# TorbenHellriegel/Speaker-Recognition-x-vectors

Hardware: AMD Instinct MI355X
Metric: x-vector embeddings/sec (300-frame utt) (higher is better)
Workload: dtype f32; 1 GPU; configs[1]: 1xMI355X batch=256 fixed 300-frame x 24-MFCC utterances, fp32 frame-level stack, extract_x_vec layer 6, random-init weights seed 42; build=xvec_hip gfx950 build a1dbbf885613, batch_per_gpu=256, frames=300

## Files before the change

### speaker-recognition-x-vectors_amd/csrc/tdnn_layer_impl.h

```cpp
#pragma once
#include <cstdlib>

#include "tdnn_common.h"

namespace xvec {

constexpr int kBM = 128, kBN = 128;
constexpr int kStageFloats = (kBM + kBN) * kBK;
constexpr int kConstFloats = 3 * kBN;
constexpr int kLdsBytes = (2 * kStageFloats + kConstFloats) * 4;

#ifdef XVEC_DIAG
static __device__ unsigned long long g_diag[8 * 8192];
#endif

struct Ctx {
    __amdgpu_buffer_rsrc_t xrsrc;
    __amdgpu_buffer_rsrc_t wrsrc;
    int x_base;
    int ur0, ur1, ur2, ur3;
    int xo0, xo1, xo2, xo3;
    int w_toff;
    __amdgpu_buffer_rsrc_t wfrsrc;
    int wf_voff;
// ... 218 lines not shown
    }

#define XV_CHUNK3(P_, N_, IT_)                                                                            \
    {                                                                                                     \
        const float* S = smem + P_ * kStageFloats;                                                        \
        const float* Sn = smem + N_ * kStageFloats;                                                       \
        XV_G3(0, gb0_0, XV_FRG_L(0, 0, S), XV_FRG_L(1, 0, S), XV_FRG_L(2, 0, S), XV_FRG_L(3, 0, S))       \
        XV_G3(0, gb0_1, XV_LST3(0, N_), XV_LST3(1, N_), XV_LST3(2, N_), XV_LST3(3, N_))                   \
        XV_G3(1, gb0_0, XV_FRG_A(0, 1, 0, S), XV_FRG_A(1, 1, 0, S), XV_FRG_A(2, 1, 0, S),                 \
              XV_FRG_A(3, 1, 0, S))                                                                       \
        XV_ADVANCE                                                                                        \
        XV_G3(0, gb1_0, XV_FRG_L(0, 1, S), XV_FRG_L(1, 1, S), XV_FRG_L(2, 1, S), XV_FRG_L(3, 1, S))       \
        XV_G3(0, gb1_1, XV_GLB3(0, (IT_) + 1), XV_GLD_A(0, 0) XV_GLD_A(1, 0),                             \
              XV_GLD_A(2, 0) XV_GLD_A(3, 0), XV_GLD_B(0, 0) XV_GLD_B(1, 0))                               \
        XV_G3(1, gb1_0, XV_FRG_A(0, 2, 0, S), XV_FRG_A(1, 2, 0, S), XV_FRG_A(2, 2, 0, S),                 \
              XV_FRG_A(3, 2, 0, S))                                                                       \
        XV_G3(0, gb2_0, XV_FRG_L(0, 2, S), XV_FRG_L(1, 2, S), XV_FRG_L(2, 2, S), XV_FRG_L(3, 2, S))       \
        XV_G3(0, gb2_1, XV_GLB3(1, (IT_) + 1), XV_GLD_B(2, 0) XV_GLD_B(3, 0), XV_NOP, XV_NOP)             \
        XV_G3(1, gb2_0, XV_FRG_A(0, 3, 0, S), XV_FRG_A(1, 3, 0, S), XV_FRG_A(2, 3, 0, S),                 \
              XV_FRG_A(3, 3, 0, S))                                                                       \
        XV_G3(0, gb3_0, XV_FRG_L(0, 3, S), XV_FRG_L(1, 3, S), XV_FRG_L(2, 3, S), XV_FRG_L(3, 3, S))       \
        XV_G3(0, gb3_1, XV_GLB3(2, (IT_) + 1), XV_NOP, XV_NOP, XV_NOP)                                    \
        __syncthreads();                      \
        XV_G3(1, gb3_0, XV_FRG_A(0, 0, 0, Sn), XV_FRG_A(1, 0, 0, Sn), XV_FRG_A(2, 0, 0, Sn),              \
              XV_FRG_A(3, 0, 0, Sn))                                                                      \
        XV_GLB3(3, (IT_) + 1)                                                                             \
    }

struct Regs {
    float4 sA0_0, sA1_0, sA2_0, sA3_0, sB0_0, sB1_0, sB2_0, sB3_0;
    float4 sA0_1, sA1_1, sA2_1, sA3_1, sB0_1, sB1_1, sB2_1, sB3_1;
    float4 fa0_0, fa1_0, fa2_0, fa3_0, fb_0, fa0_1, fa1_1, fa2_1, fa3_1, fb_1;
    float4 gb0_0, gb1_0, gb2_0, gb3_0, gb0_1, gb1_1, gb2_1, gb3_1;
    float4 w3[2][6];
};

struct Lane {
    int h, sw, a_rd, b_rd, st_off, r0, c, col;
    int st3, rd3;
};

constexpr int kPlaneBytes = kBM * kBK * 2;

__device__ __forceinline__ void s3_store(char* B, int st3, int i, const float4& v) {
    u32x2 hi, mid, lo;
    split3(v, hi, mid, lo);
    *reinterpret_cast<u32x2*>(B + st3 + i * 32 * 64) = hi;
    *reinterpret_cast<u32x2*>(B + kPlaneBytes + st3 + i * 32 * 64) = mid;
    *reinterpret_cast<u32x2*>(B + 2 * kPlaneBytes + st3 + i * 32 * 64) = lo;
}

template <int NG>
__device__ __forceinline__ void s3_gld(const TdnnArgs& a, const Ctx& cx, float4& d0, float4& d1, float4& d2, float4& d3) {
    const int soff = ((cx.tap * a.tap_rows) * a.ldx + cx.kc * kBK) * 4;
    const int rs = 32 * a.ldx * 4;
    if constexpr (NG > 0) d0 = buf_load16(cx.xrsrc, cx.xo0, soff);
    if constexpr (NG > 1) d1 = buf_load16(cx.xrsrc, cx.xo1, soff + rs);
    if constexpr (NG > 2) d2 = buf_load16(cx.xrsrc, cx.xo2, soff + 2 * rs);
    if constexpr (NG > 3) d3 = buf_load16(cx.xrsrc, cx.xo3, soff + 3 * rs);
}

__device__ __forceinline__ void s3_wld(const Ctx& cx, float4* w, int c, int n_chunks) {
    if (c >= n_chunks) c -= n_chunks;
#pragma unroll
    for (int j = 0; j < 6; ++j) w[j] = buf_load16(cx.wfrsrc, cx.wf_voff, (6 * c + j) * 1024);
}

#define XV_S3_CHUNK(P_, N_, IT_)                                                                          \
    {                                                                                                     \
        const char* S = reinterpret_cast<const char*>(smem) + P_ * kStageFloats * 4;                      \
        char* Sn = reinterpret_cast<char*>(smem) + N_ * kStageFloats * 4;                                 \
        if constexpr (G > 0) s3_store(Sn, ln.st3, 0, rg.sA0_##N_);                                         \
        if constexpr (G > 1) s3_store(Sn, ln.st3, 1, rg.sA1_##N_);                                         \
        if constexpr (G > 2) s3_store(Sn, ln.st3, 2, rg.sA2_##N_);                                         \
        if constexpr (G > 3) s3_store(Sn, ln.st3, 3, rg.sA3_##N_);                                         \
        advance<GUARD, false>(a, cx, n_chunks);                                                           \
        s3_gld<G>(a, cx, rg.sA0_##N_, rg.sA1_##N_, rg.sA2_##N_, rg.sA3_##N_);                              \
        s3_wld(cx, rg.w3[N_], (IT_) + 1, n_chunks);                                                       \
        _Pragma("unroll") for (int s3 = 0; s3 < 2; ++s3) {                                                \
            const int rd = ln.rd3 ^ (32 * s3);                                                            \
            float4 xf[4][3];                                                                              \
            _Pragma("unroll") for (int i = 0; i < G; ++i)                                                 \
                _Pragma("unroll") for (int pl = 0; pl < 3; ++pl)                                          \
                    xf[i][pl] = *reinterpret_cast<const float4*>(S + pl * kPlaneBytes + i * 32 * 64 + rd); \
            if constexpr (G > 0) s3_mfma6(acc0, xf[0], rg.w3[P_] + 3 * s3);                                \
            if constexpr (G > 1) s3_mfma6(acc1, xf[1], rg.w3[P_] + 3 * s3);                                \
            if constexpr (G > 2) s3_mfma6(acc2, xf[2], rg.w3[P_] + 3 * s3);                                \
            if constexpr (G > 3) s3_mfma6(acc3, xf[3], rg.w3[P_] + 3 * s3);                                \
        }                                                                                                 \
        __syncthreads();                      \
    }

template <int GUARD, bool INBF, bool X3, bool S3>
__device__ __forceinline__ void block_prologue(const TdnnArgs& a, float* smem, Ctx& cx, Regs& rg, const Lane& ln,
                                               int n_chunks) {
    constexpr int G = 4;
    constexpr int ES = INBF ? 2 : 4, BKE = 128 / ES;
    const int h = ln.h, sw = ln.sw, a_rd = ln.a_rd, b_rd = ln.b_rd, st_off = ln.st_off, c = ln.c;
    if constexpr (S3) {
        char* B0 = reinterpret_cast<char*>(smem);
        s3_gld<4>(a, cx, rg.sA0_0, rg.sA1_0, rg.sA2_0, rg.sA3_0);
        advance<GUARD, false>(a, cx, n_chunks);
        s3_gld<4>(a, cx, rg.sA0_1, rg.sA1_1, rg.sA2_1, rg.sA3_1);
        s3_wld(cx, rg.w3[0], 0, n_chunks);
        s3_store(B0, ln.st3, 0, rg.sA0_0);
        s3_store(B0, ln.st3, 1, rg.sA1_0);
        s3_store(B0, ln.st3, 2, rg.sA2_0);
        s3_store(B0, ln.st3, 3, rg.sA3_0);
        advance<GUARD, false>(a, cx, n_chunks);
        s3_gld<4>(a, cx, rg.sA0_0, rg.sA1_0, rg.sA2_0, rg.sA3_0);
        __syncthreads();
        return;
    }
    if constexpr (X3) {
        XV_GLD_ALL(0)
        SB();
        XV_LST3(0, 0) XV_LST3(1, 0) XV_LST3(2, 0) XV_LST3(3, 0)
        SB();
        advance<GUARD, X3>(a, cx, n_chunks);
        XV_GLD_ALL(0)
    } else {
        XV_GLD_ALL(0)
        advance<GUARD, X3>(a, cx, n_chunks);
        XV_GLD_ALL(1)
        SB();
        XV_LST_ALL(0)
        SB();
        advance<GUARD, X3>(a, cx, n_chunks);
        XV_GLD_ALL(0)
    }
    __syncthreads();
    XV_FRG_A(0, 0, 0, smem) XV_FRG_A(1, 0, 0, smem) XV_FRG_A(2, 0, 0, smem) XV_FRG_A(3, 0, 0, smem)
    XV_FRG_B(0, 0, smem)
    XV_GLB(0, 0, 0) XV_GLB(1, 0, 0) XV_GLB(2, 0, 0) XV_GLB(3, 0, 0)
    XV_GLB(0, 1, 1) XV_GLB(1, 1, 1) XV_GLB(2, 1, 1) XV_GLB(3, 1, 1)
    XV_GLB3(0, 0) XV_GLB3(1, 0) XV_GLB3(2, 0) XV_GLB3(3, 0)
    SB();
}

template <int G, int GUARD, bool POOL, bool STORE, bool INBF, bool OUTBF, bool X3, bool S3>
__device__ __forceinline__ void process_tile(const TdnnArgs& a, float* smem, Ctx& cx, Regs& rg, const Lane& ln,
                                             int64_t g0, int n0, int n_chunks) {
    constexpr int ES = INBF ? 2 : 4, BKE = 128 / ES;
    const int h = ln.h, sw = ln.sw, a_rd = ln.a_rd, b_rd = ln.b_rd, st_off = ln.st_off, c = ln.c;
    constexpr bool SWAP = INBF && OUTBF && !X3 && STORE && !POOL;
    f32x16 acc0, acc1, acc2, acc3;
    const float* cstw = smem + 2 * kStageFloats + (ln.col - n0 - (int)(threadIdx.x & 31)) + 4 * ln.h;
    if constexpr (SWAP) {
#pragma unroll
        for (int gq = 0; gq < 4; ++gq) {
            const float4 b4 = *reinterpret_cast<const float4*>(cstw + 8 * gq);
            acc0[4 * gq] = b4.x; acc0[4 * gq + 1] = b4.y; acc0[4 * gq + 2] = b4.z; acc0[4 * gq + 3] = b4.w;
        }
        acc1 = acc0; acc2 = acc0; acc3 = acc0;
    } else if constexpr (POOL) {
        const float b0 = smem[2 * kStageFloats + kBN + (ln.col - n0)];
#pragma unroll
        for (int e = 0; e < 16; ++e) acc0[e] = b0;
        acc1 = acc0; acc2 = acc0; acc3 = acc0;
    } else {
#pragma unroll
        for (int e = 0; e < 16; ++e) { acc0[e] = 0.f; acc1[e] = 0.f; acc2[e] = 0.f; acc3[e] = 0.f; }
    }

#ifdef XVEC_DIAG
    SB();
    const unsigned long long dt0 = __builtin_amdgcn_s_memtime();
    SB();
#endif
    for (int it = 0; it < n_chunks; it += 2) {
        if constexpr (S3) {
            XV_S3_CHUNK(0, 1, it)
            XV_S3_CHUNK(1, 0, it + 1)
        } else if constexpr (X3) {
            XV_CHUNK3(0, 1, it)
            XV_CHUNK3(1, 0, it + 1)
        } else {
            XV_CHUNK(0, 1, it)
            XV_CHUNK(1, 0, it + 1)
        }
    }
#ifdef XVEC_DIAG
    SB();
    const unsigned long long dt1 = __builtin_amdgcn_s_memtime();
    SB();
#endif

    const int64_t m0 = g0 * 32;
    const int col = ln.col;
    float* cst = smem + 2 * kStageFloats + (col - n0);
    const float bi = cst[0], sc = cst[kBN], sh = cst[2 * kBN];
    float negk = sh;
    if constexpr (POOL) {
        if (!cx.pivot_set) {
            const float piv = lower_half(fmaxf(acc0[0] + bi, 0.f));
            const float bmk = bi - piv;
            negk = bmk - bi;
#pragma unroll
            for (int e = 0; e < 16; ++e) {
                acc0[e] += bmk;
                if constexpr (G > 1) acc1[e] += bmk;
                if constexpr (G > 2) acc2[e] += bmk;
                if constexpr (G > 3) acc3[e] += bmk;
            }
            cst[kBN] = bmk;
            cst[2 * kBN] = negk;
            cx.pivot_set = true;
        }
    }
    const int esz = OUTBF ? 2 : 4;
    __amdgpu_buffer_rsrc_t yrsrc;
    int y_voff = 0;
    __amdgpu_buffer_rsrc_t yrsrc_lo;
    if (STORE) {
        yrsrc = make_rsrc(static_cast<char*>(a.Y) + (m0 * (int64_t)a.ldy + n0) * esz);
        if constexpr (X3 && OUTBF)
            yrsrc_lo = make_rsrc(static_cast<char*>(a.Y) + a.y_plane_bytes + (m0 * (int64_t)a.ldy + n0) * esz);
        y_voff = (4 * h * a.ldy + (col - n0)) * esz;
    }
#define XV_EPI(i_)                                                                                        \
    if constexpr (G > i_) {                                                                               \
                                                                                       \
        if constexpr (!POOL) {                                                                            \
            _Pragma("unroll") for (int e = 0; e < 16; ++e)                                                \
                acc##i_[e] = fmaf(fmaxf(acc##i_[e] + bi, 0.f), sc, sh);                                   \
            asm volatile("" : "+v"(acc##i_));                                                             \
        }                                                                                                 \
        if (STORE) {                                                                                      \
            _Pragma("unroll") for (int e = 0; e < 16; ++e) {                                              \
                const int soff = (i_ * 32 + (e & 3) + 8 * (e >> 2)) * a.ldy * esz;                        \
// ... 43 lines not shown
    }
#endif
}

template <int GUARD, bool POOL, bool STORE, bool INBF, bool OUTBF, bool X3, bool S3>
__device__ __forceinline__ void tdnn_body(const TdnnArgs& a, float* smem) {
#ifdef XVEC_DIAG
    const unsigned long long t_entry = __builtin_amdgcn_s_memtime(), r_entry = __builtin_amdgcn_s_memrealtime();
    if (threadIdx.x == 0 && blockIdx.x < 8192) { g_diag[blockIdx.x * 8 + 3] = 0; g_diag[blockIdx.x * 8 + 4] = 0; g_diag[blockIdx.x * 8 + 5] = 0; }
#endif
    const int lid = xcd_remap(blockIdx.x, gridDim.x);
    const int j = lid % a.n_tiles;
    const int p = lid / a.n_tiles;
    int64_t g_begin, g_end;
    group_range(a, p, g_begin, g_end);
    const int n0 = j * kBN;
    const int n_chunks = a.n_taps * a.cpt;

    const int tid = threadIdx.x;
    const int lane = tid & 63, wave = tid >> 6;
    Lane ln;
    ln.h = lane >> 5;
    const int r = lane & 31;
    ln.c = tid & 7;
    ln.r0 = tid >> 3;
    ln.st_off = ln.r0 * kBK + ((ln.c ^ ((ln.r0 >> 1) & 7)) << 2);
    ln.sw = (r >> 1) & 7;
    ln.a_rd = r * kBK;
    ln.b_rd = kBM * kBK + (wave * 32 + r) * kBK;
    ln.col = n0 + wave * 32 + r;
    ln.st3 = ln.r0 * 64 + ((((ln.c >> 1) ^ ((ln.r0 >> 2) & 3)) * 16) | ((ln.c & 1) * 8));
    ln.rd3 = r * 64 + ((ln.h ^ ((r >> 2) & 3)) * 16);
    if (tid < kBN) {
        smem[2 * kStageFloats + tid] = a.bias[n0 + tid];
        smem[2 * kStageFloats + kBN + tid] = POOL ? 0.f : a.scale[n0 + tid];
        smem[2 * kStageFloats + 2 * kBN + tid] = POOL ? 0.f : a.shift[n0 + tid];
    }

    Ctx cx;
    cx.g_s = g_begin;
    cx.g_end = g_end;
    cx.m0 = g_begin * 32;
    constexpr int ES = INBF ? 2 : 4;
    cx.es = ES;
    cx.xrsrc = x_rsrc<GUARD>(a, cx);
    cx.wrsrc = make_rsrc(static_cast<const char*>(a.W) + (int64_t)n0 * a.k_pad * ES);
    cx.x_base = ln.r0 * a.ldx * ES + ln.c * 16;
    cx.w_toff = ln.r0 * a.k_pad * ES + ln.c * 16;
    cx.r0 = ln.r0;
    if (INBF) {
        const int64_t ct = n0 / 32 + wave;
        cx.wfrsrc = make_rsrc(static_cast<const char*>(a.Wf) + ct * (int64_t)(a.k_pad / 16) * 1024);
        cx.wf_voff = lane * 16;
    }
    if (S3) {
        const int64_t ct = n0 / 32 + wave;
        cx.wfrsrc = make_rsrc(static_cast<const char*>(a.Wf) + ct * (int64_t)(a.k_pad / 16) * 3072);
        cx.wf_voff = lane * 16;
    }
    cx.u_tile = __builtin_amdgcn_readfirstlane(utt_of_row(a.out_map, cx.m0));
    cx.off_next = row_off(a.out_map, cx.u_tile + 1);
    if (POOL) {
        cx.pool.u = cx.u_tile;
        cx.pool.end = cx.off_next;
    }
    cx.pivot_set = false;
    set_tile_rows(a, cx);
    cx.tap = 0;
    cx.kc = 0;
    cx.itl = 0;

    Regs rg;
    block_prologue<GUARD, INBF, X3, S3>(a, smem, cx, rg, ln, n_chunks);
    int64_t g = g_begin;
    for (; g + 4 <= g_end; g += 4) process_tile<4, GUARD, POOL, STORE, INBF, OUTBF, X3, S3>(a, smem, cx, rg, ln, g, n0, n_chunks);
    const int rem = (int)(g_end - g);
    if (rem == 3) process_tile<3, GUARD, POOL, STORE, INBF, OUTBF, X3, S3>(a, smem, cx, rg, ln, g, n0, n_chunks);
    else if (rem == 2) process_tile<2, GUARD, POOL, STORE, INBF, OUTBF, X3, S3>(a, smem, cx, rg, ln, g, n0, n_chunks);
    else if (rem == 1) process_tile<1, GUARD, POOL, STORE, INBF, OUTBF, X3, S3>(a, smem, cx, rg, ln, g, n0, n_chunks);
#ifdef XVEC_DIAG
    if (threadIdx.x == 0 && blockIdx.x < 8192) {
        __builtin_amdgcn_s_waitcnt(0);
        unsigned long long* d = g_diag + blockIdx.x * 8;
        d[0] = t_entry;
        d[1] = __builtin_amdgcn_s_memtime();
        d[2] = (unsigned long long)(g_end - g_begin);
        d[6] = r_entry;
        d[7] = __builtin_amdgcn_s_memrealtime();
    }
#endif
}

template <typename K>
static hipError_t launch_kernel(K kern, const TdnnArgs& a, hipStream_t s, LdsOptIn& opt) {
    if (a.groups_total <= 0 || a.blocks_per_col <= 0 || a.blocks_per_col > a.groups_total || (a.cpt & 1))
        return hipErrorInvalidValue;
    if (hipError_t e = opt.ensure(reinterpret_cast<const void*>(kern), kLdsBytes); e != hipSuccess) return e;
    const int grid = a.blocks_per_col * a.n_tiles;
    kern<<<dim3(grid), dim3(256), kLdsBytes, s>>>(a);
    return hipGetLastError();
}

}
```

### speaker-recognition-x-vectors_amd/csrc/tdnn_split3.hip

```cpp
#include "tdnn_layer_impl.h"

namespace xvec {

template <bool POOL, bool STORE>
__global__ __launch_bounds__(256, 2) void tdnn_split3_kernel(const TdnnArgs a) {
    extern __shared__ __attribute__((aligned(16))) float smem[];
    tdnn_body<false, POOL, STORE, false, false, false, true>(a, smem);
}

hipError_t launch_tdnn_split3(const TdnnArgs& a, bool pool, hipStream_t s) {
    static LdsOptIn opt_store, opt_pool;
    if (a.n_taps != 1) return hipErrorInvalidValue;
    return pool ? launch_kernel(tdnn_split3_kernel<true, false>, a, s, opt_pool)
                : launch_kernel(tdnn_split3_kernel<false, true>, a, s, opt_store);
}

}
```

### speaker-recognition-x-vectors_amd/csrc/xvec_api.hip

```cpp
#include <hip/hip_runtime.h>

#include <algorithm>
#include <cstdio>
#include <cstdlib>
#include <cstring>
#include <new>

#include "../../include/xvec_hip.h"
#include "host_support.h"
#include "pool_segments.h"
#include "tdnn_common.h"
#include "xvec_internal.h"

using namespace xvec;

namespace {

thread_local ErrorChannel g_err;

#define HIP_TRY(expr)                                                                         \
    do {                                                                                      \
        hipError_t e_ = (expr);                                                               \
        if (e_ != hipSuccess)                                                                 \
            return g_err.fail(XVEC_ERR_HIP, "%s failed: %s (%s:%d)", #expr,                   \
                              hipGetErrorString(e_), __FILE__, __LINE__);                     \
    } while (0)

const int kCtxLen[XVEC_NUM_TDNN] = {5, 3, 3, 1, 1};
const int kCtxDil[XVEC_NUM_TDNN] = {1, 2, 3, 0, 0};

enum { T_L1 = 0, T_POOL = 5, T_SEG6 = 6, T_SEG7 = 7, T_OUT = 8, T_PACK = 9, T_COUNT = 10 };
constexpr int kMaxUtts = 65535;
constexpr int kSplit3MinRowsPerCu = 64;
constexpr int kWinoS3MinRowsPerCu = 64;

struct Policy {
    int blocks_per_cu;
    bool pp;
    int pp_min_tenths;
    int pp_cu_pct;
    bool wino;
    bool split3;
    int split3_min_rows;
    bool wino_split3;
    int wino_s3_min_rows;
};

int env_int(const char* name, int unset) {
    const char* e = getenv(name);
    return e ? atoi(e) : unset;
}

Policy read_policy() {
    const int tenths = env_int("XVEC_PP_MIN_TENTHS", 18), s3_rows = env_int("XVEC_SPLIT3_MIN_ROWS", kSplit3MinRowsPerCu);
    const int ws3_rows = env_int("XVEC_WINO_SPLIT3_MIN_ROWS", kWinoS3MinRowsPerCu);
    return {std::max(1, env_int("XVEC_BLOCKS_PER_CU", 2)), env_int("XVEC_PP", 1) != 0, tenths > 0 ? tenths : 18,
            env_int("XVEC_PP_CU_PCT", 0), env_int("XVEC_WINOGRAD", 1) != 0, env_int("XVEC_SPLIT3", 1) != 0,
            s3_rows >= 0 ? s3_rows : kSplit3MinRowsPerCu, env_int("XVEC_WINO_SPLIT3", 1) != 0,
            ws3_rows >= 0 ? ws3_rows : kWinoS3MinRowsPerCu};
}

struct DeviceGuard {
    int prev = -1;
    bool changed = false;
    hipError_t enter(int dev) {
        hipError_t e = hipGetDevice(&prev);
        if (e != hipSuccess) return e;
        if (prev != dev) {
            e = hipSetDevice(dev);
            changed = e == hipSuccess;
        }
        return e;
    }
    ~DeviceGuard() {
        if (changed) (void)hipSetDevice(prev);
    }
};

}

struct xvec_handle {
    xvec_cfg cfg;
    int cin_pad;
    TdnnGeom geo[XVEC_NUM_TDNN];
    TdnnGeom geo16[XVEC_NUM_TDNN];
    void* Wp16[XVEC_NUM_TDNN];
    void* Wp16b;
    void* Wr16[XVEC_NUM_TDNN];
    void* Wp48[XVEC_NUM_TDNN];
    void* Wr48[XVEC_NUM_TDNN];
    float* Wp[XVEC_NUM_TDNN];
    float* Wu[XVEC_NUM_TDNN];
    void* Wu3[XVEC_NUM_TDNN];
    void* Wp3[XVEC_NUM_TDNN];
    float* vec[XVEC_NUM_TDNN];
    float* Wraw[XVEC_NUM_TDNN];
    float* braw[XVEC_NUM_TDNN];
    float* vec16[XVEC_NUM_TDNN];
    bool folded[XVEC_NUM_TDNN];
    hipEvent_t load_evt[XVEC_NUM_TDNN];
    bool tdnn_loaded[XVEC_NUM_TDNN];
    float* affW[3];
    float* affB[3];
    void* affW3[3];
    int affN[3], affK[3];
    bool aff_loaded[3];
    int64_t* offs_pinned[2];
    hipEvent_t offs_evt[2];
    bool offs_pending[2];
    int offs_next;
    int num_cu;
    Policy pol;
    int last_kernel[XVEC_NUM_TDNN];
    int last_form[XVEC_NUM_TDNN];
    int last_operands[XVEC_NUM_TDNN];
    int last_aff_form[3];
    int last_aff_ranges[3];
    bool profiling;
    hipEvent_t ev0[T_COUNT], ev1[T_COUNT];
    bool ev_used[T_COUNT];
};

namespace {

struct Plan {
    int64_t total, m_pad, rows_alloc;
    size_t xpad, x16, actA, actB, act5, part, part_cnt, pooled, seg6, seg7, offs, bytes;
    int64_t part_slots;
};


Plan make_plan(const xvec_handle* h, int64_t total, int B) {
    Plan p;
    p.total = total;
    p.m_pad = round_up64(total > 0 ? total : 1, 128);
    p.rows_alloc = p.m_pad + kRowPadTail;
    const int nh = h->geo[0].n_pad, n5 = h->geo[4].n_pad;
    size_t o = 0;
    p.xpad = o;   o += align256((size_t)p.rows_alloc * h->cin_pad * 4);
    p.x16 = o;    o += align256((size_t)p.rows_alloc * h->cin_pad * 2 * 2);
    p.actA = o;   o += align256((size_t)p.rows_alloc * nh * 4);
    p.actB = o;   o += align256((size_t)p.rows_alloc * nh * 4);
    p.act5 = o;   o += align256((size_t)p.rows_alloc * (n5 > nh ? n5 : nh) * 4);
    p.part_slots = std::max<int64_t>(p.m_pad / 32 + B + 1, 2 * ((int64_t)h->num_cu + B) + 2);
// ... 57 lines not shown
    for (int i = 0; i < 3; ++i) {
        f(&h->affW[i], (size_t)h->affN[i] * h->affK[i] * 4);
        f(&h->affB[i], (size_t)h->affN[i] * 4);
        f(&h->affW3[i], h->affK[i] % 4 == 0 ? (size_t)h->affN[i] * h->affK[i] * 4 : 0);
    }
}

int aff_index(int which) { return which == XVEC_SEG6 ? 0 : which == XVEC_SEG7 ? 1 : which == XVEC_OUTPUT ? 2 : -1; }

struct StageTimer {
    xvec_handle* h;
    int idx;
    hipStream_t s;
    StageTimer(xvec_handle* h_, int idx_, hipStream_t s_) : h(h_), idx(idx_), s(s_) {
        if (h->profiling) (void)hipEventRecord(h->ev0[idx], s);
    }
    ~StageTimer() {
        if (h->profiling) {
            (void)hipEventRecord(h->ev1[idx], s);
            h->ev_used[idx] = true;
        }
    }
};

int pp_blocks_per_col(const xvec_handle* h, int n_pad, int64_t rows_out) {
    const Policy& pol = h->pol;
    if (!pol.pp || n_pad % 256 != 0) return 0;
    int bpc = h->num_cu / (n_pad / 256);
    if (pol.pp_cu_pct > 0 && pol.pp_cu_pct < 100) bpc = (bpc * pol.pp_cu_pct + 50) / 100;
    const int64_t units = (rows_out + 63) / 64;
    return (bpc >= 1 && units >= bpc && 10 * units >= pol.pp_min_tenths * (int64_t)bpc) ? bpc : 0;
}

void persistent_grid(const xvec_handle* h, int n_tiles, int64_t groups_total, int* blocks_per_col, int* pair_period) {
    const int per_col = (int)std::max<int64_t>(1, std::min<int64_t>((int64_t)h->num_cu * h->pol.blocks_per_cu / n_tiles, groups_total));
    const int nwg = per_col * n_tiles;
    const bool ok = h->pol.blocks_per_cu == 2 && nwg == 2 * h->num_cu && nwg % 16 == 0 && (nwg / 8) % (2 * n_tiles) == 0;
    *blocks_per_col = per_col;
    *pair_period = ok ? (nwg / 8) / n_tiles : 0;
}

struct LayerCall {
    int layer;
    TdnnMode mode;
    const void* X;
    int ldx;
    int64_t x_rows;
    void* X16;
    int64_t x_plane, y_plane;
    void* Y;
    float* part;
    int* part_cnt;
    RowMap map;
    int64_t rows_out;
};

enum class Launch { kDirect, kPp16, kFirst, kFirst3, kSplit3, kWino, kWinoS3 };

struct LayerPlan {
    int layer;
    Launch launch;
    int kernel, form;
    int operands;
    TdnnMode mode;
    TdnnArgs a;
    int64_t pool_units;
    int pool_bpc;
};

int plan_layer(const xvec_handle* h, const LayerCall& c, LayerPlan& lp) {
    const int l = c.layer;
    const bool bf = c.mode.prec != Prec::kF32, x3 = c.mode.prec == Prec::kBf16x3, pool = c.mode.dst == Dst::kPool;
    const bool from_act = c.mode.src == Src::kAct;
    const TdnnGeom& g = bf ? h->geo16[l] : h->geo[l];
    memset(&lp, 0, sizeof(lp));
    lp.layer = l;
    lp.mode = c.mode;
    lp.kernel = XVEC_KERNEL_TILE128;
    lp.form = XVEC_FORM_DIRECT;
    lp.operands = !bf ? XVEC_OPERANDS_FP32 : x3 ? XVEC_OPERANDS_BF16X3 : XVEC_OPERANDS_BF16;
    TdnnArgs& a = lp.a;
    a.X = c.X;
    a.W = h->Wp[l];
    a.Wf = x3 ? h->Wp48[l] : h->Wp16[l];
    const float* vecs = (bf && !x3) ? h->vec16[l] : h->vec[l];
    a.bias = vecs;
    a.scale = vecs + g.n_pad;
    a.shift = vecs + 2 * g.n_pad;
    a.Y = c.Y;
    a.x_rows = c.x_rows;
    a.ldx = c.ldx;
    a.ldy = g.n_pad;
    a.n_taps = g.n_taps;
    a.tap_rows = g.tap_rows;
    a.kpt = g.kpt;
    a.cpt = g.kpt_pad / (bf ? 2 * kBK : kBK);
    a.k_pad = x3 ? 2 * g.k_pad : g.k_pad;
    a.n_tiles = g.n_pad / 128;
    a.groups_total = (c.rows_out + 31) / 32;
    persistent_grid(h, a.n_tiles, a.groups_total, &a.blocks_per_col, &a.pair_period);
    a.pool_part = c.part;
    a.pool_cnt = c.part_cnt;
    a.out_map = c.map;
    a.span = h->geo[l].ctx_span;
    a.terms = x3 ? 2 : 1;
    a.y_plane_bytes = x3 ? (int)c.y_plane : 0;
    int bpc = 0;
    if (bf && l > 0 && from_act && c.mode.dst != Dst::kF32 && (bpc = pp_blocks_per_col(h, g.n_pad, c.rows_out))) {
        lp.launch = Launch::kPp16;
        lp.kernel = XVEC_KERNEL_PP;
        a.W = x3 ? h->Wr48[l] : h->Wr16[l];
        a.n_tiles = g.n_pad / 256;
        a.blocks_per_col = lp.pool_bpc = bpc;
        a.groups_total = lp.pool_units = (c.rows_out + 63) / 64;
        a.pair_period = 0;
    } else if (bf && l == 0 && !from_act && c.mode.dst == Dst::kAct && h->pol.pp &&
               (x3 ? tdnn_first3_applicable(a) : tdnn_first_applicable(a))) {
        lp.launch = x3 ? Launch::kFirst3 : Launch::kFirst;
        lp.kernel = XVEC_KERNEL_FIRST;
        if (!x3) a.Wf = h->Wp16b;
    } else if (x3 && c.mode.src == Src::kRows32) {
        if (!c.X16) return g_err.fail(XVEC_ERR_STATE, "internal: bf16x3 layer 1 from fp32 rows needs the streaming kernel's shapes");
        lp.mode.src = Src::kRows16;
        a.X = c.X16;
    } else if (!bf && from_act && h->pol.split3 && h->Wp3[l] && c.rows_out >= (int64_t)h->pol.split3_min_rows * h->num_cu) {
        lp.launch = Launch::kSplit3;
        lp.form = XVEC_FORM_BF16_SPLIT3;
        lp.operands = XVEC_OPERANDS_BF16_SPLIT3;
        a.terms = 3;
        a.Wf = h->Wp3[l];
    } else if (!bf && from_act && !pool && h->pol.wino && h->Wu[l] && tdnn_wino_applicable(g, c.ldx)) {
        lp.launch = Launch::kWino;
        lp.form = XVEC_FORM_WINOGRAD_F23;
        a.W = h->Wu[l];
        a.k_pad = 4 * g.kpt_pad;
        a.p_fixed = c.map.offsets ? 0 : wino_pair_count(c.map.fixed_T - c.map.cum, g.tap_rows);
        const int64_t pairs = c.map.offsets ? (c.rows_out >> 1) + (int64_t)c.map.n_utts * g.tap_rows
                                            : (int64_t)c.map.n_utts * a.p_fixed;
        a.groups_total = (pairs + 31) / 32;
        persistent_grid(h, a.n_tiles, a.groups_total, &a.blocks_per_col, &a.pair_period);
        if (h->pol.wino_split3 && h->Wu3[l] && tdnn_wino_s3_applicable(g, c.ldx) &&
            c.rows_out >= (int64_t)h->pol.wino_s3_min_rows * h->num_cu) {
            lp.launch = Launch::kWinoS3;
            lp.operands = XVEC_OPERANDS_BF16_SPLIT3;
            a.Wf = h->Wu3[l];
        }
    }
    const bool rows32 = lp.mode.src == Src::kRows32;
    const int64_t x_plane = x3 && !rows32 ? c.x_plane : 0;
    if (x3) {
        a.x_plane_bytes = (int)x_plane;
        a.x_bytes = c.x_rows > 0 && !rows32 ? x_plane + c.x_rows * (int64_t)c.ldx * 2 : 0;
    }
    const int64_t es = (bf && !rows32) ? 2 : 4;
    if (((int64_t)c.map.n_utts * a.span + kRowPadTail) * c.ldx * es + x_plane > 0x7fffffff)
        return g_err.fail(XVEC_ERR_TOO_LARGE, "layer %d: %d utterances x %d channels exceed 32-bit row offsets; split the batch",
                          l, c.map.n_utts, c.ldx);
    if (x3 && (x_plane > 0x3fffffff || c.y_plane > 0x3fffffff))
        return g_err.fail(XVEC_ERR_TOO_LARGE, "batch too large for bf16x3 (plane offsets must fit 30 bits); split it");
    if (pool && lp.launch != Launch::kPp16 &&
        (size_t)((c.rows_out + 31) / 32 + c.map.n_utts + 1) * 3 * g.n_pad * 4 > 0x7fffffffull)
        return g_err.fail(XVEC_ERR_TOO_LARGE, "batch too large: pooling partials exceed 2 GiB; split it");
    return XVEC_OK;
}

int launch_layer(xvec_handle* h, const LayerPlan& lp, hipStream_t s) {
    StageTimer t(h, T_L1 + lp.layer, s);
    const bool pool = lp.mode.dst == Dst::kPool;
    switch (lp.launch) {
        case Launch::kPp16: HIP_TRY(launch_tdnn_pp16(lp.a, pool, s)); break;
        case Launch::kFirst: HIP_TRY(launch_tdnn_first(lp.a, h->num_cu, s)); break;
        case Launch::kFirst3: HIP_TRY(launch_tdnn_first3(lp.a, h->num_cu, s)); break;
        case Launch::kSplit3: HIP_TRY(launch_tdnn_split3(lp.a, pool, s)); break;
// ... 260 lines not shown
                             un ? un + 2 * npp : nullptr));
    return XVEC_OK;
}

}

extern "C" {

const char* xvec_last_error(void) { return g_err.c_str(); }
#ifndef XVEC_BUILD_ID
#define XVEC_BUILD_ID "unknown"
#endif
const char* xvec_version(void) { return "xvec_hip gfx950 build " XVEC_BUILD_ID; }

int xvec_create(const xvec_cfg* cfg, xvec_handle** out) {
    if (!cfg || !out) return g_err.fail(XVEC_ERR_ARG, "null argument");
    if (cfg->input_size < 1 || cfg->hidden_size < 1 || cfg->num_classes < 1 || cfg->x_vector_size < 1)
        return g_err.fail(XVEC_ERR_ARG, "sizes must be positive");
    if (cfg->hidden_size > 8192 || cfg->input_size > 8192)
        return g_err.fail(XVEC_ERR_ARG, "input_size / hidden_size above 8192 are not supported (32-bit row offsets)");
    DeviceGuard guard;
    HIP_TRY(guard.enter(cfg->device));
    hipDeviceProp_t prop;
    HIP_TRY(hipGetDeviceProperties(&prop, cfg->device));
    if (strncmp(prop.gcnArchName, "gfx950", 6) != 0)
        return g_err.fail(XVEC_ERR_STATE, "device %d is %s; this library is built for gfx950 only", cfg->device,
                          prop.gcnArchName);
    xvec_handle* h = new (std::nothrow) xvec_handle();
    if (!h) return g_err.fail(XVEC_ERR_STATE, "out of host memory");
    memset(h, 0, sizeof(*h));
    h->cfg = *cfg;
    h->num_cu = device_cu_count();
    h->pol = read_policy();
    h->cin_pad = round_up(cfg->input_size, 4);
    fill_geometry(h, h->geo, 2 * kBK);
    fill_geometry(h, h->geo16, 4 * kBK);
    const int N[3] = {cfg->x_vector_size, cfg->x_vector_size, cfg->num_classes};
    const int K[3] = {2 * XVEC_POOL_CHANNELS, cfg->x_vector_size, cfg->x_vector_size};
    std::copy(N, N + 3, h->affN);
    std::copy(K, K + 3, h->affK);
    bool ok = true;
    each_weight_buffer(h, [&](auto** ptr, size_t bytes) {
        ok = ok && (bytes == 0 || hipMalloc(reinterpret_cast<void**>(ptr), bytes) == hipSuccess);
    });
    if (!ok) {
        xvec_destroy(h);
        return g_err.fail(XVEC_ERR_HIP, "hipMalloc of packed weights failed");
    }
    for (int i = 0; i < 2 && ok; ++i)
        ok = hipEventCreateWithFlags(&h->offs_evt[i], hipEventDisableTiming) == hipSuccess &&
             hipHostMalloc(reinterpret_cast<void**>(&h->offs_pinned[i]), (size_t)(kMaxUtts + 1) * 8,
                           hipHostMallocDefault) == hipSuccess;
    for (int i = 0; i < T_COUNT && ok; ++i)
        ok = hipEventCreate(&h->ev0[i]) == hipSuccess && hipEventCreate(&h->ev1[i]) == hipSuccess;
    for (int i = 0; i < XVEC_NUM_TDNN && ok; ++i)
        ok = hipEventCreateWithFlags(&h->load_evt[i], hipEventDisableTiming) == hipSuccess;
    if (!ok) {
        xvec_destroy(h);
        return g_err.fail(XVEC_ERR_HIP, "hipEventCreate / hipHostMalloc failed");
    }
    *out = h;
    return XVEC_OK;
}

void xvec_destroy(xvec_handle* h) {
    if (!h) return;
// ... 451 lines not shown
```

### speaker-recognition-x-vectors_amd/csrc/xvec_internal.h

```cpp
#pragma once
#include <hip/hip_runtime.h>
#include <stddef.h>
#include <stdint.h>
#include "affine_plan.h"

namespace xvec {

constexpr int kBK = 32;
constexpr int kRowPadTail = 264;

inline int round_up(int v, int m) { return (v + m - 1) / m * m; }
inline int64_t round_up64(int64_t v, int64_t m) { return (v + m - 1) / m * m; }

struct RowMap {
    const int64_t* offsets;
    int n_utts;
    int fixed_T;
    int cum;
};
#ifdef __HIPCC__
__device__ __forceinline__ int64_t row_off(const RowMap& m, int u) {
    return (m.offsets ? m.offsets[u] : (int64_t)u * m.fixed_T) - (int64_t)u * m.cum;
}
__device__ __forceinline__ int utt_of_row(const RowMap& m, int64_t p) {
// ... 45 lines not shown
struct TdnnArgs {
    const void* X;
    const void* W;
    const void* Wf;
    const float* bias;
    const float* scale;
    const float* shift;
    void* Y;
    int64_t x_rows;
    int ldx, ldy;
    int n_taps, tap_rows, kpt, cpt;
    int k_pad;
    int n_tiles;
    int blocks_per_col;
    int64_t groups_total;
    int pair_period;
    RowMap out_map;
    int span;
    int p_fixed;
    float* pool_part;
    int* pool_cnt;
    int terms;
    int x_plane_bytes;
    int y_plane_bytes;
    int64_t x_bytes;
};

enum class Prec { kF32, kBf16, kBf16x3 };
enum class Src { kRows32, kRows16, kAct };
enum class Dst { kAct, kF32, kPool };
struct TdnnMode { Prec prec; Src src; Dst dst; };
hipError_t launch_tdnn(const TdnnArgs& a, TdnnMode m, hipStream_t s);
hipError_t launch_tdnn_split3(const TdnnArgs& a, bool pool, hipStream_t s);
hipError_t launch_tdnn_pp16(const TdnnArgs& a, bool pool, hipStream_t s);
bool tdnn_first_applicable(const TdnnArgs& a);
hipError_t launch_patch_bias_kslots(const float* bias, const TdnnGeom& geo, void* Wf16, hipStream_t s);
hipError_t launch_tdnn_first(const TdnnArgs& a, int num_cu, hipStream_t s);
bool tdnn_first3_applicable(const TdnnArgs& a);
hipError_t launch_tdnn_first3(const TdnnArgs& a, int num_cu, hipStream_t s);
hipError_t launch_pack_tdnn_split3(const float* W, const TdnnGeom& geo, void* Wf3, hipStream_t s);
hipError_t launch_pack_tdnn_rows_bf16(const float* W, const float* in_scale, const TdnnGeom& geo, void* Wr16, hipStream_t s);
hipError_t launch_fold_bias(const float* W, const float* bias, const float* in_shift, const TdnnGeom& geo, float* vec16,
                            hipStream_t s);
hipError_t launch_pack_tdnn_rows_bf16x3(const float* W, const TdnnGeom& geo, void* Wr48, hipStream_t s);

bool tdnn_wino_applicable(const TdnnGeom& g, int ldx);
hipError_t launch_tdnn_wino(const TdnnArgs& a, hipStream_t s);
bool tdnn_wino_s3_applicable(const TdnnGeom& g, int ldx);
hipError_t launch_tdnn_wino_s3(const TdnnArgs& a, hipStream_t s);
hipError_t launch_pack_wino(const float* W, const TdnnGeom& geo, float* Wu, hipStream_t s);
hipError_t launch_pack_wino_split3(const float* W, const TdnnGeom& geo, void* Wu3, hipStream_t s);

struct PoolArgs {
    const float* X;
    float* out;
    const int32_t* lengths;
    int B, T, C;
};
hipError_t launch_stat_pool(const PoolArgs& a, hipStream_t s);

struct PoolFinalizeArgs {
    const float* part;
    const int* cnt;
    int64_t units_total;
    int blocks_per_col;
    float* out;
// ... 28 lines not shown
```

Measured before the change: 150,200 embeddings/s.

## Restructure split3 TDNN pipeline to raise occupancy to three blocks per CU

The split3 (bf16x3) TDNN kernel drops its double-buffered register staging for activations and weights and interleaves LDS fragment reads with MFMAs one item at a time, reloading weight halves as they are consumed. The LDS layout is resized to the exact three-plane buffers and launch bounds go to 3 blocks per CU, with a runtime occupancy query choosing the persistent grid size. The aim is to cut register and LDS footprint so more waves hide latency, at the cost of shorter prefetch distance for global loads. The pooling pivot is also truncated to bf16 precision.

Result: faster. 154,600 embeddings/s, median of 6 (+2.9%).

```diff
diff --git a/speaker-recognition-x-vectors_amd/csrc/tdnn_layer_impl.h b/speaker-recognition-x-vectors_amd/csrc/tdnn_layer_impl.h
--- a/speaker-recognition-x-vectors_amd/csrc/tdnn_layer_impl.h
+++ b/speaker-recognition-x-vectors_amd/csrc/tdnn_layer_impl.h
@@ -274,7 +274,7 @@
     float4 sA0_1, sA1_1, sA2_1, sA3_1, sB0_1, sB1_1, sB2_1, sB3_1;
     float4 fa0_0, fa1_0, fa2_0, fa3_0, fb_0, fa0_1, fa1_1, fa2_1, fa3_1, fb_1;
     float4 gb0_0, gb1_0, gb2_0, gb3_0, gb0_1, gb1_1, gb2_1, gb3_1;
-    float4 w3[2][6];
+    float4 w3[6];
 };
 
 struct Lane {
@@ -283,6 +283,10 @@
 };
 
 constexpr int kPlaneBytes = kBM * kBK * 2;
+constexpr int kS3BufBytes = 3 * kPlaneBytes;
+constexpr int kS3LdsBytes = 2 * kS3BufBytes + kConstFloats * 4;
+template <bool S3>
+constexpr int kCstFloat = S3 ? 2 * kS3BufBytes / 4 : 2 * kStageFloats;
 
 __device__ __forceinline__ void s3_store(char* B, int st3, int i, const float4& v) {
     u32x2 hi, mid, lo;
@@ -302,34 +306,43 @@
     if constexpr (NG > 3) d3 = buf_load16(cx.xrsrc, cx.xo3, soff + 3 * rs);
 }
 
-__device__ __forceinline__ void s3_wld(const Ctx& cx, float4* w, int c, int n_chunks) {
+__device__ __forceinline__ void s3_wld(const Ctx& cx, float4* w, int c, int s, int n_chunks) {
     if (c >= n_chunks) c -= n_chunks;
 #pragma unroll
-    for (int j = 0; j < 6; ++j) w[j] = buf_load16(cx.wfrsrc, cx.wf_voff, (6 * c + j) * 1024);
-}
-
+    for (int j = 0; j < 3; ++j) w[3 * s + j] = buf_load16(cx.wfrsrc, cx.wf_voff, (6 * c + 3 * s + j) * 1024);
+}
+
+__device__ __forceinline__ void s3_frag(const char* S, int rd3, int i, int s, float4* xf) {
+#pragma unroll
+    for (int pl = 0; pl < 3; ++pl)
+        xf[pl] = *reinterpret_cast<const float4*>(S + pl * kPlaneBytes + i * 32 * 64 + (rd3 ^ (32 * s)));
+}
+
+template <int G, int N>
+__device__ __forceinline__ void s3_item(const Ctx& cx, const char* S, int rd3, f32x16& acc, float4 (&xf)[2][3], float4* w,
+                                        int c_next, int n_chunks) {
+    constexpr int s = N / G, i = N % G;
+    if constexpr (N + 1 < 2 * G) s3_frag(S, rd3, (N + 1) % G, (N + 1) / G, xf[(N + 1) & 1]);
+    s3_mfma6(acc, xf[N & 1], w + 3 * s);
+    if constexpr (i == G - 1) s3_wld(cx, w, c_next, s, n_chunks);
+}
+
+#define XV_S3_ITEM(i_, s_, IT_)                                                                           \
+    if constexpr (G > i_) { s3_item<G, s_ * G + i_>(cx, S, ln.rd3, acc##i_, xf, rg.w3, (IT_) + 1, n_chunks); SB(); }
 #define XV_S3_CHUNK(P_, N_, IT_)                                                                          \
     {                                                                                                     \
-        const char* S = reinterpret_cast<const char*>(smem) + P_ * kStageFloats * 4;                      \
-        char* Sn = reinterpret_cast<char*>(smem) + N_ * kStageFloats * 4;                                 \
-        if constexpr (G > 0) s3_store(Sn, ln.st3, 0, rg.sA0_##N_);                                         \
-        if constexpr (G > 1) s3_store(Sn, ln.st3, 1, rg.sA1_##N_);                                         \
-        if constexpr (G > 2) s3_store(Sn, ln.st3, 2, rg.sA2_##N_);                                         \
-        if constexpr (G > 3) s3_store(Sn, ln.st3, 3, rg.sA3_##N_);                                         \
+        const char* S = reinterpret_cast<const char*>(smem) + P_ * kS3BufBytes;                           \
+        char* Sn = reinterpret_cast<char*>(smem) + N_ * kS3BufBytes;                                      \
+        float4 xf[2][3];                                                                                  \
+        s3_frag(S, ln.rd3, 0, 0, xf[0]);                                                                  \
+        if constexpr (G > 0) s3_store(Sn, ln.st3, 0, rg.sA0_0);                                           \
+        if constexpr (G > 1) s3_store(Sn, ln.st3, 1, rg.sA1_0);                                           \
+        if constexpr (G > 2) s3_store(Sn, ln.st3, 2, rg.sA2_0);                                           \
+        if constexpr (G > 3) s3_store(Sn, ln.st3, 3, rg.sA3_0);                                           \
         advance<GUARD, false>(a, cx, n_chunks);                                                           \
-        s3_gld<G>(a, cx, rg.sA0_##N_, rg.sA1_##N_, rg.sA2_##N_, rg.sA3_##N_);                              \
-        s3_wld(cx, rg.w3[N_], (IT_) + 1, n_chunks);                                                       \
-        _Pragma("unroll") for (int s3 = 0; s3 < 2; ++s3) {                                                \
-            const int rd = ln.rd3 ^ (32 * s3);                                                            \
-            float4 xf[4][3];                                                                              \
-            _Pragma("unroll") for (int i = 0; i < G; ++i)                                                 \
-                _Pragma("unroll") for (int pl = 0; pl < 3; ++pl)                                          \
-                    xf[i][pl] = *reinterpret_cast<const float4*>(S + pl * kPlaneBytes + i * 32 * 64 + rd); \
-            if constexpr (G > 0) s3_mfma6(acc0, xf[0], rg.w3[P_] + 3 * s3);                                \
-            if constexpr (G > 1) s3_mfma6(acc1, xf[1], rg.w3[P_] + 3 * s3);                                \
-            if constexpr (G > 2) s3_mfma6(acc2, xf[2], rg.w3[P_] + 3 * s3);                                \
-            if constexpr (G > 3) s3_mfma6(acc3, xf[3], rg.w3[P_] + 3 * s3);                                \
-        }                                                                                                 \
+        s3_gld<G>(a, cx, rg.sA0_0, rg.sA1_0, rg.sA2_0, rg.sA3_0);                                         \
+        XV_S3_ITEM(0, 0, IT_) XV_S3_ITEM(1, 0, IT_) XV_S3_ITEM(2, 0, IT_) XV_S3_ITEM(3, 0, IT_)           \
+        XV_S3_ITEM(0, 1, IT_) XV_S3_ITEM(1, 1, IT_) XV_S3_ITEM(2, 1, IT_) XV_S3_ITEM(3, 1, IT_)           \
         __syncthreads();                      \
     }
 
@@ -342,9 +355,8 @@
     if constexpr (S3) {
         char* B0 = reinterpret_cast<char*>(smem);
         s3_gld<4>(a, cx, rg.sA0_0, rg.sA1_0, rg.sA2_0, rg.sA3_0);
-        advance<GUARD, false>(a, cx, n_chunks);
-        s3_gld<4>(a, cx, rg.sA0_1, rg.sA1_1, rg.sA2_1, rg.sA3_1);
-        s3_wld(cx, rg.w3[0], 0, n_chunks);
+        s3_wld(cx, rg.w3, 0, 0, n_chunks);
+        s3_wld(cx, rg.w3, 0, 1, n_chunks);
         s3_store(B0, ln.st3, 0, rg.sA0_0);
         s3_store(B0, ln.st3, 1, rg.sA1_0);
         s3_store(B0, ln.st3, 2, rg.sA2_0);
@@ -387,7 +399,7 @@
     const int h = ln.h, sw = ln.sw, a_rd = ln.a_rd, b_rd = ln.b_rd, st_off = ln.st_off, c = ln.c;
     constexpr bool SWAP = INBF && OUTBF && !X3 && STORE && !POOL;
     f32x16 acc0, acc1, acc2, acc3;
-    const float* cstw = smem + 2 * kStageFloats + (ln.col - n0 - (int)(threadIdx.x & 31)) + 4 * ln.h;
+    const float* cstw = smem + kCstFloat<S3> + (ln.col - n0 - (int)(threadIdx.x & 31)) + 4 * ln.h;
     if constexpr (SWAP) {
 #pragma unroll
         for (int gq = 0; gq < 4; ++gq) {
@@ -396,7 +408,7 @@
         }
         acc1 = acc0; acc2 = acc0; acc3 = acc0;
     } else if constexpr (POOL) {
-        const float b0 = smem[2 * kStageFloats + kBN + (ln.col - n0)];
+        const float b0 = smem[kCstFloat<S3> + kBN + (ln.col - n0)];
 #pragma unroll
         for (int e = 0; e < 16; ++e) acc0[e] = b0;
         acc1 = acc0; acc2 = acc0; acc3 = acc0;
@@ -430,14 +442,14 @@
 
     const int64_t m0 = g0 * 32;
     const int col = ln.col;
-    float* cst = smem + 2 * kStageFloats + (col - n0);
+    float* cst = smem + kCstFloat<S3> + (col - n0);
     const float bi = cst[0], sc = cst[kBN], sh = cst[2 * kBN];
     float negk = sh;
     if constexpr (POOL) {
         if (!cx.pivot_set) {
-            const float piv = lower_half(fmaxf(acc0[0] + bi, 0.f));
+            const float piv = __uint_as_float(__float_as_uint(lower_half(fmaxf(acc0[0] + bi, 0.f))) & 0xffff0000u);
             const float bmk = bi - piv;
-            negk = bmk - bi;
+            negk = -piv;
 #pragma unroll
             for (int e = 0; e < 16; ++e) {
                 acc0[e] += bmk;
@@ -547,9 +559,9 @@
     ln.st3 = ln.r0 * 64 + ((((ln.c >> 1) ^ ((ln.r0 >> 2) & 3)) * 16) | ((ln.c & 1) * 8));
     ln.rd3 = r * 64 + ((ln.h ^ ((r >> 2) & 3)) * 16);
     if (tid < kBN) {
-        smem[2 * kStageFloats + tid] = a.bias[n0 + tid];
-        smem[2 * kStageFloats + kBN + tid] = POOL ? 0.f : a.scale[n0 + tid];
-        smem[2 * kStageFloats + 2 * kBN + tid] = POOL ? 0.f : a.shift[n0 + tid];
+        smem[kCstFloat<S3> + tid] = a.bias[n0 + tid];
+        smem[kCstFloat<S3> + kBN + tid] = POOL ? 0.f : a.scale[n0 + tid];
+        smem[kCstFloat<S3> + 2 * kBN + tid] = POOL ? 0.f : a.shift[n0 + tid];
     }
 
     Ctx cx;
@@ -607,12 +619,12 @@
 }
 
 template <typename K>
-static hipError_t launch_kernel(K kern, const TdnnArgs& a, hipStream_t s, LdsOptIn& opt) {
+static hipError_t launch_kernel(K kern, const TdnnArgs& a, hipStream_t s, LdsOptIn& opt, int lds_bytes = kLdsBytes) {
     if (a.groups_total <= 0 || a.blocks_per_col <= 0 || a.blocks_per_col > a.groups_total || (a.cpt & 1))
         return hipErrorInvalidValue;
-    if (hipError_t e = opt.ensure(reinterpret_cast<const void*>(kern), kLdsBytes); e != hipSuccess) return e;
+    if (hipError_t e = opt.ensure(reinterpret_cast<const void*>(kern), lds_bytes); e != hipSuccess) return e;
     const int grid = a.blocks_per_col * a.n_tiles;
-    kern<<<dim3(grid), dim3(256), kLdsBytes, s>>>(a);
+    kern<<<dim3(grid), dim3(256), lds_bytes, s>>>(a);
     return hipGetLastError();
 }
 
diff --git a/speaker-recognition-x-vectors_amd/csrc/tdnn_split3.hip b/speaker-recognition-x-vectors_amd/csrc/tdnn_split3.hip
--- a/speaker-recognition-x-vectors_amd/csrc/tdnn_split3.hip
+++ b/speaker-recognition-x-vectors_amd/csrc/tdnn_split3.hip
@@ -3,16 +3,32 @@
 namespace xvec {
 
 template <bool POOL, bool STORE>
-__global__ __launch_bounds__(256, 2) void tdnn_split3_kernel(const TdnnArgs a) {
+__global__ __launch_bounds__(256, 3) void tdnn_split3_kernel(const TdnnArgs a) {
     extern __shared__ __attribute__((aligned(16))) float smem[];
     tdnn_body<false, POOL, STORE, false, false, false, true>(a, smem);
 }
 
+static LdsOptIn opt_store, opt_pool;
+
 hipError_t launch_tdnn_split3(const TdnnArgs& a, bool pool, hipStream_t s) {
-    static LdsOptIn opt_store, opt_pool;
     if (a.n_taps != 1) return hipErrorInvalidValue;
-    return pool ? launch_kernel(tdnn_split3_kernel<true, false>, a, s, opt_pool)
-                : launch_kernel(tdnn_split3_kernel<false, true>, a, s, opt_store);
+    return pool ? launch_kernel(tdnn_split3_kernel<true, false>, a, s, opt_pool, kS3LdsBytes)
+                : launch_kernel(tdnn_split3_kernel<false, true>, a, s, opt_store, kS3LdsBytes);
+}
+
+hipError_t tdnn_split3_max_blocks_per_cu(int* blocks) {
+    const void* kern[2] = {reinterpret_cast<const void*>(tdnn_split3_kernel<false, true>),
+                           reinterpret_cast<const void*>(tdnn_split3_kernel<true, false>)};
+    LdsOptIn* opt[2] = {&opt_store, &opt_pool};
+    int least = 0;
+    for (int v = 0; v < 2; ++v) {
+        int n = 0;
+        if (hipError_t e = opt[v]->ensure(kern[v], kS3LdsBytes); e != hipSuccess) return e;
+        if (hipError_t e = hipOccupancyMaxActiveBlocksPerMultiprocessor(&n, kern[v], 256, kS3LdsBytes); e != hipSuccess) return e;
+        least = v == 0 ? n : (n < least ? n : least);
+    }
+    *blocks = least;
+    return hipSuccess;
 }
 
 }
diff --git a/speaker-recognition-x-vectors_amd/csrc/xvec_api.hip b/speaker-recognition-x-vectors_amd/csrc/xvec_api.hip
--- a/speaker-recognition-x-vectors_amd/csrc/xvec_api.hip
+++ b/speaker-recognition-x-vectors_amd/csrc/xvec_api.hip
@@ -54,7 +54,7 @@
 Policy read_policy() {
     const int tenths = env_int("XVEC_PP_MIN_TENTHS", 18), s3_rows = env_int("XVEC_SPLIT3_MIN_ROWS", kSplit3MinRowsPerCu);
     const int ws3_rows = env_int("XVEC_WINO_SPLIT3_MIN_ROWS", kWinoS3MinRowsPerCu);
-    return {std::max(1, env_int("XVEC_BLOCKS_PER_CU", 2)), env_int("XVEC_PP", 1) != 0, tenths > 0 ? tenths : 18,
+    return {std::max(0, env_int("XVEC_BLOCKS_PER_CU", 0)), env_int("XVEC_PP", 1) != 0, tenths > 0 ? tenths : 18,
             env_int("XVEC_PP_CU_PCT", 0), env_int("XVEC_WINOGRAD", 1) != 0, env_int("XVEC_SPLIT3", 1) != 0,
             s3_rows >= 0 ? s3_rows : kSplit3MinRowsPerCu, env_int("XVEC_WINO_SPLIT3", 1) != 0,
             ws3_rows >= 0 ? ws3_rows : kWinoS3MinRowsPerCu};
@@ -110,6 +110,7 @@
     bool offs_pending[2];
     int offs_next;
     int num_cu;
+    int split3_blocks_cu;
     Policy pol;
     int last_kernel[XVEC_NUM_TDNN];
     int last_form[XVEC_NUM_TDNN];
@@ -233,10 +234,15 @@
     return (bpc >= 1 && units >= bpc && 10 * units >= pol.pp_min_tenths * (int64_t)bpc) ? bpc : 0;
 }
 
-void persistent_grid(const xvec_handle* h, int n_tiles, int64_t groups_total, int* blocks_per_col, int* pair_period) {
-    const int per_col = (int)std::max<int64_t>(1, std::min<int64_t>((int64_t)h->num_cu * h->pol.blocks_per_cu / n_tiles, groups_total));
+int blocks_per_cu(const xvec_handle* h, bool split3) {
+    const int holds = split3 ? h->split3_blocks_cu : 2;
+    return h->pol.blocks_per_cu > 0 ? std::min(h->pol.blocks_per_cu, holds) : holds;
+}
+
+void persistent_grid(const xvec_handle* h, int per_cu, int n_tiles, int64_t groups_total, int* blocks_per_col, int* pair_period) {
+    const int per_col = (int)std::max<int64_t>(1, std::min<int64_t>((int64_t)h->num_cu * per_cu / n_tiles, groups_total));
     const int nwg = per_col * n_tiles;
-    const bool ok = h->pol.blocks_per_cu == 2 && nwg == 2 * h->num_cu && nwg % 16 == 0 && (nwg / 8) % (2 * n_tiles) == 0;
+    const bool ok = per_cu == 2 && nwg == 2 * h->num_cu && nwg % 16 == 0 && (nwg / 8) % (2 * n_tiles) == 0;
     *blocks_per_col = per_col;
     *pair_period = ok ? (nwg / 8) / n_tiles : 0;
 }
@@ -299,7 +305,7 @@
     a.k_pad = x3 ? 2 * g.k_pad : g.k_pad;
     a.n_tiles = g.n_pad / 128;
     a.groups_total = (c.rows_out + 31) / 32;
-    persistent_grid(h, a.n_tiles, a.groups_total, &a.blocks_per_col, &a.pair_period);
+    persistent_grid(h, blocks_per_cu(h, false), a.n_tiles, a.groups_total, &a.blocks_per_col, &a.pair_period);
     a.pool_part = c.part;
     a.pool_cnt = c.part_cnt;
     a.out_map = c.map;
@@ -330,6 +336,7 @@
         lp.operands = XVEC_OPERANDS_BF16_SPLIT3;
         a.terms = 3;
         a.Wf = h->Wp3[l];
+        persistent_grid(h, blocks_per_cu(h, true), a.n_tiles, a.groups_total, &a.blocks_per_col, &a.pair_period);
     } else if (!bf && from_act && !pool && h->pol.wino && h->Wu[l] && tdnn_wino_applicable(g, c.ldx)) {
         lp.launch = Launch::kWino;
         lp.form = XVEC_FORM_WINOGRAD_F23;
@@ -339,7 +346,7 @@
         const int64_t pairs = c.map.offsets ? (c.rows_out >> 1) + (int64_t)c.map.n_utts * g.tap_rows
                                             : (int64_t)c.map.n_utts * a.p_fixed;
         a.groups_total = (pairs + 31) / 32;
-        persistent_grid(h, a.n_tiles, a.groups_total, &a.blocks_per_col, &a.pair_period);
+        persistent_grid(h, blocks_per_cu(h, false), a.n_tiles, a.groups_total, &a.blocks_per_col, &a.pair_period);
         if (h->pol.wino_split3 && h->Wu3[l] && tdnn_wino_s3_applicable(g, c.ldx) &&
             c.rows_out >= (int64_t)h->pol.wino_s3_min_rows * h->num_cu) {
             lp.launch = Launch::kWinoS3;
@@ -666,6 +673,12 @@
     h->cfg = *cfg;
     h->num_cu = device_cu_count();
     h->pol = read_policy();
+    int s3_blocks = 0;
+    if (hipError_t e = tdnn_split3_max_blocks_per_cu(&s3_blocks); e != hipSuccess) {
+        delete h;
+        return g_err.fail(XVEC_ERR_HIP, "occupancy query of tdnn_split3_kernel failed: %s", hipGetErrorString(e));
+    }
+    h->split3_blocks_cu = std::max(1, std::min(3, s3_blocks));
     h->cin_pad = round_up(cfg->input_size, 4);
     fill_geometry(h, h->geo, 2 * kBK);
     fill_geometry(h, h->geo16, 4 * kBK);
diff --git a/speaker-recognition-x-vectors_amd/csrc/xvec_internal.h b/speaker-recognition-x-vectors_amd/csrc/xvec_internal.h
--- a/speaker-recognition-x-vectors_amd/csrc/xvec_internal.h
+++ b/speaker-recognition-x-vectors_amd/csrc/xvec_internal.h
@@ -101,6 +101,7 @@
 struct TdnnMode { Prec prec; Src src; Dst dst; };
 hipError_t launch_tdnn(const TdnnArgs& a, TdnnMode m, hipStream_t s);
 hipError_t launch_tdnn_split3(const TdnnArgs& a, bool pool, hipStream_t s);
+hipError_t tdnn_split3_max_blocks_per_cu(int* blocks);
 hipError_t launch_tdnn_pp16(const TdnnArgs& a, bool pool, hipStream_t s);
 bool tdnn_first_applicable(const TdnnArgs& a);
 hipError_t launch_patch_bias_kslots(const float* bias, const TdnnGeom& geo, void* Wf16, hipStream_t s);
```
